# OpenSpaceAI/Nesie

Measured on AMD Instinct MI355X. Metric: ScanNet scenes/sec (fwd+bwd, 40k pts, bs=8), higher is better.
Workload: dtype f32; 1 GPU; Nesie-VoteNet supervised pretrain step (nesie-votenet-scannet-pretrain-10%): fwd+bwd+AdamW, 40000 pts/scene, fp32, random-init weights; scenes_per_gpu=8, global_batch=8, parallelism=single, world_size=1, hip_graph=True, deterministic_backward=True, index_chain_pipelined=True, forward_cu_budget=232, forward_cu_budget_from_the_head_on=248, grad_allreduce_bytes=10561936, resident_input_scenes=0

## Files before the change

nesie_amd/csrc/pwconv.hip:

```cpp
#include <algorithm>
#include "pwconv_fwd.h"
#include <stdlib.h>

namespace nesie {
PW_GEOM_DECL(4, 1, 4, 1, 1)
PW_GEOM_DECL(4, 1, 4, 1, 2)
PW_GEOM_DECL(8, 1, 4, 1, 1)
PW_GEOM_DECL(8, 1, 8, 1, 1)
PW_GEOM_DECL(9, 1, 8, 1, 1)
PW_GEOM_DECL(8, 2, 8, 1, 1)
PW_GEOM_DECL(9, 2, 8, 1, 1)
PW_GEOM_DECL(8, 4, 8, 1, 1)
int pw_launch_sparse_8_1_8_1_1(const PwFwd &a, int grid, size_t lds, hipStream_t s);

__global__ __launch_bounds__(64) void pw_stats_finalize_kernel(
    int cout, int nslots, const float *__restrict__ part, const float *__restrict__ gamma,
    const float *__restrict__ beta, float *running_mean, float *running_var, float momentum,
    float eps, float *__restrict__ coef, const float *__restrict__ chan_bias) {
  const int ch = blockIdx.x, g = ch / cout, m = ch % cout;
  const float4 *pp = (const float4 *)part + ((size_t)g * nslots) * cout + m;
  double n = 0.0, mean = 0.0, m2 = 0.0;
  auto merge = [&](double nb_, double mb_, double m2b_) {
    if (nb_ <= 0.0) return;
    const double nn = n + nb_, d = mb_ - mean;
    mean += d * (nb_ / nn);
    m2 += m2b_ + d * d * (n * nb_ / nn);
    n = nn;
  };
  auto slot = [&](const float4 q) {
    if (q.x > 0.f) {
      const double ni = q.x, mi = (double)q.y + (double)q.z / ni;
      const double m2i = (double)q.w - (double)q.z * (double)q.z / ni;
      merge(ni, mi, m2i > 0.0 ? m2i : 0.0);
    }
  };
  int i = threadIdx.x;
  for (; i + 192 < nslots; i += 256) {
    float4 q[4];
#pragma unroll
    for (int u = 0; u < 4; ++u) q[u] = pp[(size_t)(i + 64 * u) * cout];
#pragma unroll
    for (int u = 0; u < 4; ++u) slot(q[u]);
  }
  for (; i < nslots; i += 64) slot(pp[(size_t)i * cout]);
#pragma unroll
  for (int off = 32; off >= 1; off >>= 1) {
    const double nb_ = __shfl_xor(n, off, 64), mb_ = __shfl_xor(mean, off, 64), m2b_ = __shfl_xor(m2, off, 64);
    const double nn = n + nb_;
    if (nn > 0.0) {
      const double d = mb_ - mean;
      const double mm = (n * mean + nb_ * mb_) / nn;
      m2 = m2 + m2b_ + d * d * (n * nb_ / nn);
      mean = mm;
    }
    n = nn;
  }
  if (threadIdx.x != 0) return;
  const double var = n > 0.0 ? m2 / n : 0.0;
  const double invstd = 1.0 / sqrt(var + (double)eps);
  if (running_mean) {
    const double shown = mean + (chan_bias ? (double)chan_bias[ch] : 0.0);
    running_mean[ch] = (float)((1.0 - momentum) * running_mean[ch] + momentum * shown);
    const double unbiased = n > 1.0 ? var * n / (n - 1.0) : var;
    running_var[ch] = (float)((1.0 - momentum) * running_var[ch] + momentum * unbiased);
  }
  const double gm = gamma ? (double)gamma[ch] : 1.0, bt = beta ? (double)beta[ch] : 0.0;
  coef[ch * 4 + 0] = (float)(gm * invstd);
  coef[ch * 4 + 1] = (float)(bt - mean * gm * invstd);
  coef[ch * 4 + 2] = (float)mean;
  coef[ch * 4 + 3] = (float)invstd;
}

__global__ __launch_bounds__(256) void pw_pool_finish_kernel(
    long long total, int channels, int ng, int groups, int nsub, int pg, const float *__restrict__ pmax,
    const float *__restrict__ pmin, const uint8_t *__restrict__ amax,
    const uint8_t *__restrict__ amin, const float *__restrict__ coef, float lo,
    float *__restrict__ pooled, uint8_t *__restrict__ arg, float *__restrict__ zstar) {
  const long long i = (long long)blockIdx.x * 256 + threadIdx.x;
  if (i >= total) return;
  const long long row = i / groups;
  const int c = (int)((row / channels) % ng) * channels + (int)(row % channels);
  const float sc = coef ? coef[c * 4 + 0] : 1.f, bi = coef ? coef[c * 4 + 1] : 0.f;
  const bool use_min = coef && sc < 0.f;
  const float *src = use_min ? pmin : pmax;
  const uint8_t *asrc = use_min ? amin : amax;
  float e = src[i * nsub];
  int at = asrc[i * nsub];
  for (int u = 1; u < nsub; ++u) {
    const float v = src[i * nsub + u];
    const bool better = use_min ? v < e : v > e;
    at = better ? u * pg + asrc[i * nsub + u] : at;
    e = better ? v : e;
  }
  pooled[i] = coef ? fmaxf(__builtin_fmaf(e, sc, bi), lo) : e;
  arg[i] = (uint8_t)at;
  if (zstar) zstar[i] = e;
}

struct PwGeom { int kt16, kh, wr, wc, rw, pt, nhalf, per_cu; };

static bool pw_geometry(int k, int cout, PwGeom *o) {
  if (k < 1 || cout < 1 || cout > 512) return false;
  if (k <= 64) { o->kt16 = 4; o->kh = 1; }
  else if (k <= 128) { o->kt16 = 8; o->kh = 1; }
  else if (k <= 144) { o->kt16 = 9; o->kh = 1; }
  else if (k <= 256) { o->kt16 = 8; o->kh = 2; }
  else if (k <= 288) { o->kt16 = 9; o->kh = 2; }
  else if (k > 384 && k <= 512) { o->kt16 = 8; o->kh = 4; }
  else return false;
  o->nhalf = (cout + 127) / 128;
  if (o->kt16 == 4) {
    o->wr = 4; o->wc = 1; o->rw = cout <= 64 ? 1 : 2;
  } else if (cout <= 64 && o->kt16 == 8 && o->kh == 1) {
    o->wr = 4; o->wc = 1; o->rw = 1;
  } else {
    o->wr = 8; o->wc = 1; o->rw = 1;
  }
  o->pt = 64 * o->wc;
  o->per_cu = pw_per_cu(o->kt16, o->kh, o->wr * o->wc, o->wc, o->rw);
  static const int one = [] { const char *e = getenv("NESIE_PW_ONE_PER_CU"); return e ? atoi(e) : 0; }();
  if (one) o->per_cu = 1;
  return true;
}

static size_t pw_lds_bytes(const PwGeom &g) { return (size_t)2 * 16 * g.kt16 * g.pt * sizeof(float); }

}

using namespace nesie;

#ifdef PW_STAMP
long long *g_pw_stamps = nullptr;
#endif

extern "C" int nesie_pw_supported(int k, int cout, long long p) {
  PwGeom g;
  return pw_geometry(k, cout, &g) && p % g.pt == 0 && (long long)(k > cout ? k : cout) * p < (1ll << 30) ? 1 : 0;
}

static int pw_groups(const PwGeom &g, int nb, int ng, long long p) {
  const long long tiles = (long long)(nb / ng) * cdiv(p, g.pt);
  long long nwg = (long long)cu_count() * g.per_cu / (ng * g.nhalf);
  if (nwg < 1) nwg = 1;
  if (nwg > tiles) nwg = tiles;
  if (g.nhalf > 1) {
    const long long unit = 8 / std::__gcd((long long)8, (long long)ng);
    const long long r = nwg / unit * unit;
    if (r > 0 && r * 10 >= nwg * 9) nwg = r;
  }
  return (int)nwg;
}

extern "C" int nesie_pw_stat_slots(int nb, int ng, int k, int cout, long long p) {
  PwGeom g;
  if (!pw_geometry(k, cout, &g) || ng < 1) return 0;
  return pw_groups(g, nb, ng, p) * g.wc;
}

#ifdef PW_DEV
PW_GEOM_DEF(8, 2, 8, 1, 1)
PW_GEOM_DEF(8, 1, 8, 1, 1)
#endif

struct PwHost { int in_relu, rb_group, pool_group, pool_min, k4_in, sp_ns; };

static int pw_forward_impl(const char *W, PwFwd a, const PwHost &h, void *stream) {
  const int nb = a.nb, ng = a.ng, k = a.k, cout = a.cout;
  const long long p = a.p;
  NESIE_REQUIRE(nb >= 0 && ng >= 1 && k >= 1 && cout >= 1 && p >= 0, W);
  if (nb == 0 || p == 0) return NESIE_OK;
  NESIE_REQUIRE(nb % ng == 0 && (a.x || a.sp_ent) && a.w, W);
  PwGeom g;
  if (!pw_geometry(k, cout, &g) || p % g.pt != 0 || (long long)(k > cout ? k : cout) * p >= (1ll << 30)) {
    set_error("%s: %d -> %d over %lld positions is outside the built tiles", W, k, cout, p);
    return NESIE_ERR_UNSUPPORTED;
  }
  NESIE_REQUIRE(((uintptr_t)a.x & 15) == 0 && (a.x_bs & 3) == 0, W);
  NESIE_REQUIRE(!a.y || (((uintptr_t)a.y & 15) == 0 && (a.y_bs & 3) == 0), W);
  int epi = 0, pg = 16;
  if (a.in_coef) epi |= PW_AFFINE;
  if (a.y) epi |= PW_STORE;
  if (a.stat_part) epi |= PW_STATS;
  if (a.row_bias) {
    NESIE_REQUIRE(h.rb_group >= 16 && (h.rb_group & (h.rb_group - 1)) == 0 && p % h.rb_group == 0, W);
    epi |= PW_ROWBIAS;
  }
  if (a.bias) epi |= PW_BIAS;
  if (a.bn_z) {
    NESIE_REQUIRE((a.y || a.k4_gpart) && a.bn_coef && a.bn_part && ((uintptr_t)a.bn_z & 15) == 0 && (a.bnz_bs & 3) == 0, W);
    epi |= PW_BNRED;
  }
  if (h.k4_in) {
    NESIE_REQUIRE(a.k4_w && a.in_coef && k == 64 && ng == 1 && a.x_bs >= 4 * p && ((uintptr_t)a.k4_w & 15) == 0, W);
    epi |= PW_K4IN;
  }
  if (a.k4_gpart) {
    NESIE_REQUIRE(a.k4_w && a.bn_z && !a.y && cout == 64 && ng == 1 && a.bnz_bs >= 4 * p && ((uintptr_t)a.k4_w & 15) == 0 &&
                  ((uintptr_t)a.k4_gpart & 15) == 0, W);
    epi |= PW_K4Z;
  }
  if (h.pool_group) {
    NESIE_REQUIRE(h.pool_group == 16 || h.pool_group == 32, W);
    NESIE_REQUIRE(a.pool_max && a.arg_max && p % h.pool_group == 0, W);
    NESIE_REQUIRE(!h.pool_min || (a.pool_min && a.arg_min), W);
    epi |= PW_POOL | (h.pool_min ? PW_POOLMIN : 0);
    pg = h.pool_group;
  }
  if (a.sp_ent) {
    NESIE_REQUIRE(k == 128 && cout % 128 == 0 && epi == (PW_STORE | PW_BNRED) && ((uintptr_t)a.sp_ent & 7) == 0, W);
    NESIE_REQUIRE((h.sp_ns == 16 || h.sp_ns == 32 || h.sp_ns == 64) && p % 64 == 0, W);
  }
  a.sp_ns_shift = a.sp_ent ? __builtin_ctz((unsigned)h.sp_ns) : 0;
  a.sp_groups = a.sp_ent ? (int)(p / h.sp_ns) : 0;
  a.in_lo = h.in_relu ? 0.f : -__builtin_inff();
  a.rb_shift = a.row_bias ? __builtin_ctz((unsigned)h.rb_group) : 0;
  a.w_stage = 1;
  a.rev = walk_dir((long long)nb * (h.k4_in ? 4 : k) * p * 4);
#ifdef PW_STAMP
  a.stamps = g_pw_stamps;
#endif
  a.tiles_per_batch = cdiv(p, g.pt);
  a.nslots = nesie_pw_stat_slots(nb, ng, k, cout, p);
  a.nwg_g = pw_groups(g, nb, ng, p);
  a.nhalf = g.nhalf;
  const int grid = a.nwg_g * ng * g.nhalf;
  static const bool xcd_on = !(getenv("NESIE_PW_XCD") && atoi(getenv("NESIE_PW_XCD")) == 0);
  a.xcd_map = (xcd_on && g.nhalf > 1 && grid % (8 * g.nhalf) == 0) ? 1 : 0;
  const size_t lds = pw_lds_bytes(g) + (a.k4_gpart ? 2048 : 0);
  hipStream_t s = (hipStream_t)stream;
  int st = NESIE_ERR_UNSUPPORTED;
#define G(KT16, KH, WR, WC, RW)                                                          \
  if (g.kt16 == KT16 && g.kh == KH && g.wr == WR && g.wc == WC && g.rw == RW)            \
  st = PW_GEOM_NAME(KT16, KH, WR, WC, RW)(a, epi, pg, grid, lds, s)
#ifdef PW_DEV
  G(8, 2, 8, 1, 1); G(8, 1, 8, 1, 1);
#else
  if (a.sp_ent) {
    st = pw_launch_sparse_8_1_8_1_1(a, grid, lds, s);
  } else {
    G(4, 1, 4, 1, 1); G(4, 1, 4, 1, 2); G(8, 1, 4, 1, 1); G(8, 1, 8, 1, 1);
    G(9, 1, 8, 1, 1); G(8, 2, 8, 1, 1); G(9, 2, 8, 1, 1); G(8, 4, 8, 1, 1);
  }
#endif
#undef G
  if (st != NESIE_OK) {
    if (st == NESIE_ERR_UNSUPPORTED && !strstr(nesie_last_error(), "epilogue"))
      set_error("%s: no build for %d -> %d", W, k, cout);
    return st;
  }
  return check_launch(W);
}

static PwFwd pw_problem(int nb, int ng, int k, int cout, long long p, const float *x, long long x_bstride,
                        const float *w) {
  PwFwd a{};
  a.nb = nb; a.ng = ng; a.k = k; a.cout = cout; a.p = p;
  a.x = x; a.x_bs = x_bstride; a.w = w;
  return a;
}

extern "C" int nesie_pw_layer_forward(int nb, int ng, int k, int cout, long long p,
                                      const float *x, long long x_bstride, const float *w,
                                      long long w_gstride, int w_rstride, int w_cstride,
                                      const float *in_coef, int in_relu, const float *row_bias,
                                      int rb_group, const float *bias, float *y,
                                      long long y_bstride, float *stat_part, int pool_group,
                                      int pool_min, float *pool_max_out, float *pool_min_out,
                                      uint8_t *arg_max_out, uint8_t *arg_min_out, void *stream) {
  PwFwd a = pw_problem(nb, ng, k, cout, p, x, x_bstride, w);
  a.w_gs = w_gstride; a.w_rs = w_rstride; a.w_cs = w_cstride;
  a.in_coef = in_coef; a.row_bias = row_bias; a.bias = bias;
  a.y = y; a.y_bs = y_bstride; a.stat_part = stat_part;
  a.pool_max = pool_max_out; a.pool_min = pool_min_out; a.arg_max = arg_max_out; a.arg_min = arg_min_out;
  PwHost h{};
  h.in_relu = in_relu; h.rb_group = rb_group; h.pool_group = pool_group; h.pool_min = pool_min;
  return pw_forward_impl("pw_layer_forward", a, h, stream);
}

extern "C" int nesie_pw_dgrad_bn_reduce(int nb, int ng, int k, int cout, long long p,
                                        const float *x, long long x_bstride, const float *w,
                                        long long w_gstride, int w_rstride, int w_cstride,
                                        float *y, long long y_bstride, const float *bn_z,
                                        long long bnz_bstride, const float *bn_coef,
                                        float *bn_part, void *stream) {
  const char *W = "pw_dgrad_bn_reduce";
  NESIE_REQUIRE(y && bn_z && bn_coef && bn_part, W);
  PwFwd a = pw_problem(nb, ng, k, cout, p, x, x_bstride, w);
  a.w_gs = w_gstride; a.w_rs = w_rstride; a.w_cs = w_cstride;
  a.y = y; a.y_bs = y_bstride;
  a.bn_z = bn_z; a.bnz_bs = bnz_bstride; a.bn_coef = bn_coef; a.bn_part = bn_part;
  return pw_forward_impl(W, a, PwHost{}, stream);
}

extern "C" int nesie_pw_dgrad_bn_reduce_sparse(int nb, int ng, int c, int cout, long long p, int ns,
                                               const float *ent, const float *w, long long w_gstride,
                                               int w_rstride, int w_cstride, float *y,
                                               long long y_bstride, const float *bn_z,
                                               long long bnz_bstride, const float *bn_coef,
                                               float *bn_part, void *stream) {
  const char *W = "pw_dgrad_bn_reduce_sparse";
  NESIE_REQUIRE(ent && y && bn_z && bn_coef && bn_part && c == 128, W);
  PwFwd a = pw_problem(nb, ng, c, cout, p, nullptr, 0, w);
  a.w_gs = w_gstride; a.w_rs = w_rstride; a.w_cs = w_cstride;
  a.y = y; a.y_bs = y_bstride;
  a.bn_z = bn_z; a.bnz_bs = bnz_bstride; a.bn_coef = bn_coef; a.bn_part = bn_part;
  a.sp_ent = (const float2 *)ent;
  PwHost h{};
  h.sp_ns = ns;
  return pw_forward_impl(W, a, h, stream);
}

extern "C" int nesie_pw_layer_forward_k4(int nb, int cout, long long p, const float *x4,
                                         long long x4_bstride, const float *w0, const float *w,
                                         int w_rstride, int w_cstride, const float *in_coef,
                                         float *y, long long y_bstride, float *stat_part,
                                         void *stream) {
  PwFwd a = pw_problem(nb, 1, 64, cout, p, x4, x4_bstride, w);
  a.w_rs = w_rstride; a.w_cs = w_cstride;
  a.in_coef = in_coef; a.k4_w = w0;
  a.y = y; a.y_bs = y_bstride; a.stat_part = stat_part;
  PwHost h{};
  h.in_relu = 1; h.k4_in = 1;
  return pw_forward_impl("pw_layer_forward_k4", a, h, stream);
}

extern "C" int nesie_pw_dgrad_bn_reduce_k4(int nb, int k, long long p, const float *x,
                                           long long x_bstride, const float *w, int w_rstride,
                                           int w_cstride, const float *x4, long long x4_bstride,
                                           const float *w0, const float *bn_coef, float *bn_part,
                                           float *g_part, void *stream) {
  const char *W = "pw_dgrad_bn_reduce_k4";
  NESIE_REQUIRE(x4 && w0 && bn_coef && bn_part && g_part, W);
  PwFwd a = pw_problem(nb, 1, k, 64, p, x, x_bstride, w);
  a.w_rs = w_rstride; a.w_cs = w_cstride;
  a.bn_z = x4; a.bnz_bs = x4_bstride; a.bn_coef = bn_coef; a.bn_part = bn_part;
  a.k4_w = w0; a.k4_gpart = g_part;
  return pw_forward_impl(W, a, PwHost{}, stream);
}

extern "C" int nesie_pw_stats_finalize(int channels, int cout, int nslots, const float *stat_part,
                                       const float *gamma, const float *beta,
                                       float *running_mean, float *running_var, float momentum,
                                       float eps, float *coef, const float *chan_bias,
                                       void *stream) {
  const char *W = "pw_stats_finalize";
  NESIE_REQUIRE(channels >= 1 && cout >= 1 && channels % cout == 0 && nslots >= 1, W);
  NESIE_REQUIRE(stat_part && coef && (running_mean == nullptr) == (running_var == nullptr), W);
  hipLaunchKernelGGL(pw_stats_finalize_kernel, dim3(channels), dim3(64), 0, (hipStream_t)stream,
                     cout, nslots, stat_part, gamma, beta, running_mean, running_var, momentum,
                     eps, coef, chan_bias);
  return check_launch(W);
}

extern "C" int nesie_pw_pool_finish(int nb, int ng, int channels, long long p, int group, int pool_group,
                                    const float *pmax, const float *pmin, const uint8_t *amax,
                                    const uint8_t *amin, const float *coef, int relu,
                                    float *pooled, uint8_t *argmax, float *zstar, void *stream) {
  const char *W = "pw_pool_finish";
  NESIE_REQUIRE(nb >= 0 && ng >= 1 && channels >= 1 && p >= 0 && group >= 1, W);
  if (nb == 0 || p == 0) return NESIE_OK;
  NESIE_REQUIRE((pool_group == 16 || pool_group == 32) && group % pool_group == 0 && p % group == 0, W);
  NESIE_REQUIRE(group <= 256 && pmax && amax && pooled && argmax && (!coef || (pmin && amin)), W);
  const long long total = (long long)nb * channels * (p / group);
  hipLaunchKernelGGL(pw_pool_finish_kernel, dim3(cdiv(total, 256)), dim3(256), 0, (hipStream_t)stream,
                     total, channels, ng, (int)(p / group), group / pool_group, pool_group, pmax, pmin,
                     amax, amin, coef, relu ? 0.f : -__builtin_inff(), pooled, argmax, zstar);
  return check_launch(W);
}
```

nesie_amd/csrc/pwconv_fwd.h:

```cpp
#pragma once
#include "common.h"
#include <stdlib.h>
#include <string.h>
#include <type_traits>

namespace nesie {

typedef float f32x4 __attribute__((ext_vector_type(4)));
typedef float f32x2 __attribute__((ext_vector_type(2)));

template <int I, int N, class F>
__device__ __forceinline__ void static_for(F &&f) {
  if constexpr (I < N) {
    f(std::integral_constant<int, I>{});
    static_for<I + 1, N>(f);
  }
}

__device__ __forceinline__ unsigned lds_addr(const void *p) {
  return (unsigned)(uintptr_t)(__attribute__((address_space(3))) const void *)p;
}

template <int OFF>
__device__ __forceinline__ f32x4 lds_read_b128(unsigned addr) {
  static_assert(OFF >= 0 && OFF < 65536, "ds_read_b128 reach");
  f32x4 v;
  asm volatile("ds_read_b128 %0, %1 offset:%2" : "=v"(v) : "v"(addr), "n"(OFF));
  return v;
}

template <int OFF>
__device__ __forceinline__ void lds_write_b128(unsigned addr, f32x4 v) {
  static_assert(OFF >= 0 && OFF < 65536, "ds_write_b128 reach");
  asm volatile("ds_write_b128 %0, %1 offset:%2" ::"v"(addr), "v"(v), "n"(OFF) : "memory");
}

__device__ __forceinline__ f32x4 load16_saddr(unsigned voff, const void *sbase) {
  return *(const f32x4 *)((const char *)sbase + voff);
}

template <int IMM>
__device__ __forceinline__ void store16_saddr(unsigned voff, f32x4 v, void *sbase) {
  *(f32x4 *)((char *)sbase + voff + IMM) = v;
}

template <int N>
__device__ __forceinline__ void lgkm_wait() {
  asm volatile("s_waitcnt lgkmcnt(%0)" ::"n"(N) : "memory");
}

enum : int {
  PW_STORE = 1,
  PW_STATS = 2,
  PW_POOL = 4,
  PW_POOLMIN = 8,
  PW_ROWBIAS = 16,
  PW_BIAS = 32,
  PW_AFFINE = 64,
  PW_BNRED = 128,
  PW_SPARSE128 = 256,
  PW_SPARSE256 = 512,
  PW_K4IN = 1024,
  PW_K4Z = 2048,
};

__device__ __forceinline__ float k4_dot(const float4 w, float x0, float x1, float x2, float x3) {
  return __builtin_fmaf(w.w, x3, __builtin_fmaf(w.z, x2, __builtin_fmaf(w.y, x1, w.x * x0)));
}

struct PwFwd {
  const float *x; long long x_bs; long long p; int nb, k;
  const float *w; long long w_gs; int w_rs, w_cs; int ng, cout;
  const float *in_coef; float in_lo;
  float *y; long long y_bs;
  const float *row_bias; int rb_shift;
  const float *bias;
  float *stat_part; int nslots;
  float *pool_max, *pool_min; uint8_t *arg_max, *arg_min;
  const float *bn_z; long long bnz_bs;
  const float *bn_coef; float *bn_part;
  int tiles_per_batch, nwg_g, nhalf;
  int xcd_map;
  const float2 *sp_ent; int sp_ns_shift, sp_groups;
  int w_stage;
  int rev;
  const float *k4_w;
  float *k4_gpart;
  long long *stamps;
};
#ifdef PW_STAMP
#define STAMP(slot)                                                                      \
  if (a.stamps && blockIdx.x == 0 && lane == 0 && (wave == 0 || wave == 4) && iter < 24) \
    a.stamps[((wave >> 2) * 24 + iter) * 8 + (slot)] = __builtin_amdgcn_s_memtime();
#define STAMP_CLK(which)                                                     \
  if (a.stamps && blockIdx.x == 0 && threadIdx.x == 0) {                      \
    a.stamps[2 * 24 * 8 + 2 * (which)] = __builtin_amdgcn_s_memtime();       \
    a.stamps[2 * 24 * 8 + 2 * (which) + 1] = __builtin_amdgcn_s_memrealtime(); \
  }
#define STAMP_WG(which)                                                                    \
  if (a.stamps && threadIdx.x == 0 && blockIdx.x < 1024)                                    \
    a.stamps[512 + blockIdx.x * 4 + (which)] = __builtin_amdgcn_s_memrealtime();
#else
#define STAMP(slot)
#define STAMP_CLK(which)
#define STAMP_WG(which)
#endif

constexpr int pw_per_cu(int kt16, int kh, int nw, int wc, int rw) {
  const int lds = 2 * 16 * kt16 * 64 * wc * 4;
  int n = 160 * 1024 / lds;
  const int cap = nw == 4 ? (kt16 * kh * rw <= 4 ? 4 : 2) : (kt16 * kh * rw <= 8 ? 2 : 1);
  return n < cap ? n : cap;
}
constexpr int pw_min_waves(int kt16, int kh, int nw, int wc, int rw) {
  return pw_per_cu(kt16, kh, nw, wc, rw) * nw / 4;
}

template <int KT16, int KH, int WR, int WC, int RW, int EPI, int PG, bool RAGGED>
__global__ __launch_bounds__(WR *WC * 64, pw_min_waves(KT16, KH, WR *WC, WC, RW))
void pw_fwd_kernel(const PwFwd a) {
  constexpr int NW = WR * WC, NT = NW * 64, KT = 16 * KT16, KQ = KT / 4, PT = 64 * WC;
  constexpr int TILE = KT * PT, CPR = PT / 4;
  constexpr int NCH = KT * CPR;
  constexpr int NX = (NCH + NT - 1) / NT;
  constexpr bool EVEN = NCH == NX * NT;
  constexpr int ROWSTEP = NT / CPR;
  constexpr int CROWS = WR * RW * 16;
  constexpr int SPC = (EPI & PW_SPARSE128) ? 128 : (EPI & PW_SPARSE256) ? 256 : 0;
  constexpr bool K4Z = (EPI & PW_K4Z) != 0;
  static_assert(SPC % ROWSTEP == 0 && (SPC == 0 || (NCH == NX * NT && SPC <= KH * KT)), "sparse rows");
  static_assert(NT % CPR == 0 && (PG == 16 || PG == 32), "tile");
  extern __shared__ __attribute__((aligned(16))) float lds[];
  STAMP_WG(0)

  const int tid = threadIdx.x, lane = tid & 63, quad = lane >> 4, l16 = lane & 15;
  const int wave = __builtin_amdgcn_readfirstlane(tid >> 6);
  const int wr = wave / WC, wc = wave % WC;
  int half, sid;
  if (a.xcd_map) {
    const int xcd = blockIdx.x & 7, slot = blockIdx.x >> 3;
    half = slot % a.nhalf;
    sid = xcd + 8 * (slot / a.nhalf);
  } else {
    half = blockIdx.x % a.nhalf;
    sid = blockIdx.x / a.nhalf;
  }
  const int g = sid % a.ng, rank = sid / a.ng;
  const int k = a.k;
  const int c0 = half * CROWS;
  const int cout = a.cout;
  const long long p = a.p;

  const int srow = tid / CPR, scol = tid % CPR;
  auto slot_row = [](int i) constexpr { return (EVEN || i + 1 < NX) ? i * ROWSTEP : KT - ROWSTEP; };
  const unsigned voff0 = (unsigned)(((size_t)srow * p + scol * 4) * 4);
  unsigned voff_last[NX];
#pragma unroll
  for (int i = 0; i < NX; ++i) {
    int row = (KH - 1) * KT + slot_row(i) + srow;
    row = row < k ? row : k - 1;
    voff_last[i] = (unsigned)(((size_t)(row - (KH - 1) * KT) * p + scol * 4) * 4);
  }
  const unsigned lw0 = lds_addr(lds) + (unsigned)((srow * PT + scol * 4) * 4);

  float wreg[RW][KH * KQ];
  const bool w_rows = KT % 64 == 0 && (a.w_stage & 1) && a.w_cs == 1 && (a.w_rs & 3) == 0 && (a.w_gs & 3) == 0 && ((uintptr_t)a.w & 15) == 0;
  if (w_rows) {
    static_assert(WR * WC * RW * 16 <= 2 * PT, "the waves' blocks fit the two operand buffers");
    constexpr int WROWS = RW * 16, C4 = KT / 4, NL = (WROWS * C4 + 63) / 64;
    float *wl = lds + wave * (WROWS * KT);
    const int m0 = c0 + wr * WROWS;
    const float *wg0 = a.w + (size_t)g * a.w_gs + (size_t)m0 * a.w_rs;
#pragma unroll
    for (int kh = 0; kh < KH; ++kh) {
#pragma unroll
      for (int i = 0; i < NL; ++i) {
        const int f = i * 64 + lane, row = f / C4, c4 = f % C4, kcol = kh * KT + 4 * c4;
        if (NL * 64 == WROWS * C4 || f < WROWS * C4) {
          f32x4 v = (f32x4){0.f, 0.f, 0.f, 0.f};
          if (m0 + row < cout) {
            const float *src = wg0 + (size_t)row * a.w_rs + kcol;
            if (kcol + 3 < k) {
              v = *(const f32x4 *)src;
            } else {
#pragma unroll
              for (int e = 0; e < 4; ++e) v[e] = kcol + e < k ? src[e] : 0.f;
            }
          }
          *(f32x4 *)(wl + row * KT + ((4 * c4) ^ (4 * (row & 15)))) = v;
        }
      }
#pragma unroll
      for (int rw = 0; rw < RW; ++rw)
#pragma unroll
        for (int kk = 0; kk < KQ; ++kk)
          wreg[rw][kh * KQ + kk] = wl[(rw * 16 + l16) * KT + ((4 * kk + quad) ^ (4 * l16))];
    }
    __syncthreads();
  } else {
#pragma unroll
    for (int rw = 0; rw < RW; ++rw) {
      const int m = c0 + (wr * RW + rw) * 16 + l16;
      const float *wg = a.w + (size_t)g * a.w_gs + (size_t)m * a.w_rs;
#pragma unroll
      for (int kk = 0; kk < KH * KQ; ++kk) {
        const int kx = 4 * kk + quad;
        wreg[rw][kk] = (m < cout && kx < k) ? wg[(size_t)kx * a.w_cs] : 0.f;
      }
    }
  }
  float2 cof[(EPI & PW_AFFINE) ? KH : 1][(EPI & PW_AFFINE) ? NX : 1];
  if (EPI & PW_AFFINE) {
#pragma unroll
    for (int kh = 0; kh < KH; ++kh)
#pragma unroll
      for (int i = 0; i < NX; ++i) {
        int row = kh * KT + slot_row(i) + srow;
// ... 46 lines not shown
      const float *x4 = a.x + (size_t)(g + a.ng * QQ(c)) * a.x_bs + (size_t)RR(c) * PT + (size_t)i * p;
      stg[i] = load16_saddr(live ? (unsigned)(scol * 16) : 0u, live ? x4 : a.x);
      return;
    }
    const float *xb = a.x + (size_t)(g + a.ng * QQ(c)) * a.x_bs + (size_t)RR(c) * PT + (long long)(kh * KT - SPC) * p;
    if constexpr (kh < KH - 1) {
      const float *xs = live ? xb + (size_t)slot_row(i) * p : a.x;
      stg[i] = load16_saddr(live ? voff0 : 0u, xs);
    } else {
      stg[i] = load16_saddr(live ? voff_last[i] : 0u, live ? xb : a.x);
    }
  };
  auto write_slot = [&](auto ic, auto khc, int buf) {
    constexpr int i = decltype(ic)::value;
    f32x4 q = stg[i];
    if constexpr ((EPI & PW_K4IN) != 0) {
#pragma unroll
      for (int e = 0; e < 4; ++e) q[e] = k4_dot(k4w[i], stg[0][e], stg[1][e], stg[2][e], stg[3][e]);
    }
    if constexpr (K4Z) {
      if constexpr (i == 0) lds_write_b128<0>(k4z_lw + (unsigned)(buf * 1024), stx);
    }
    if constexpr (SPC > 0 && decltype(khc)::value * KT + slot_row(i) < SPC) {
      const int at = __float_as_int(q[1]) - sp_pos0;
      const float v = q[0];
      q[0] = at == 0 ? v : 0.f;
      q[1] = at == 1 ? v : 0.f;
      q[2] = at == 2 ? v : 0.f;
      q[3] = at == 3 ? v : 0.f;
    } else if constexpr ((EPI & PW_AFFINE) != 0) {
      const float2 co = cof[decltype(khc)::value][i];
      const float lo = a.in_lo;
      q[0] = fmaxf(__builtin_fmaf(q[0], co.x, co.y), lo);
      q[1] = fmaxf(__builtin_fmaf(q[1], co.x, co.y), lo);
      q[2] = fmaxf(__builtin_fmaf(q[2], co.x, co.y), lo);
      q[3] = fmaxf(__builtin_fmaf(q[3], co.x, co.y), lo);
    }
    lds_write_b128<slot_row(i) * PT * 4>(lw0 + (unsigned)(buf * TILE * 4), q);
  };

  float s1[RW], s2[RW], shift[RW];
#pragma unroll
  for (int rw = 0; rw < RW; ++rw) s1[rw] = s2[rw] = shift[rw] = 0.f;
  int ntile_done = 0;
  constexpr bool PERM = !(EPI & PW_POOL) || (EPI & (PW_STORE | PW_STATS));
  constexpr int RS = PERM ? 16 : 4;
  const int q0 = wc * 64 + (PERM ? 4 : 16) * quad;
  unsigned roff[RW];
#pragma unroll
  for (int rw = 0; rw < RW; ++rw)
    roff[rw] = (unsigned)(((size_t)(c0 + (wr * RW + rw) * 16 + l16) * p + q0) * 4);

  static_assert(!K4Z || ((EPI & PW_BNRED) && !RAGGED && WC == 1), "PW_K4Z rides on PW_BNRED");
  f32x4 zv[((EPI & PW_BNRED) && !K4Z) ? RW : 1][4];
  float4 k4zw[K4Z ? RW : 1];
  float gx[K4Z ? RW : 1][4];
  float r0[RW], r1[RW];
  float4 zc[RW];
#pragma unroll
  for (int rw = 0; rw < RW; ++rw) {
    r0[rw] = r1[rw] = 0.f;
    zc[rw] = make_float4(0.f, 0.f, 0.f, 0.f);
    if (EPI & PW_BNRED) {
      const int m = c0 + (wr * RW + rw) * 16 + l16;
      if (!RAGGED || m < cout) zc[rw] = *(const float4 *)(a.bn_coef + ((size_t)g * cout + m) * 4);
      if constexpr (K4Z) {
        k4zw[rw] = *(const float4 *)(a.k4_w + (size_t)m * 4);
#pragma unroll
        for (int j = 0; j < 4; ++j) gx[rw][j] = 0.f;
      }
    }
  }
  auto row_ok = [&](int rw) { return !RAGGED || c0 + (wr * RW + rw) * 16 + l16 < cout; };
  auto load_z = [&](int n, long long p0) {
    const float *zt = a.bn_z + (size_t)n * a.bnz_bs + p0;
    if constexpr (K4Z) return;
#pragma unroll
    for (int rw = 0; rw < RW; ++rw) {
#pragma unroll
      for (int r = 0; r < 4; ++r)
        zv[rw][r] = row_ok(rw) ? load16_saddr(roff[rw] + 4u * RS * r, zt) : (f32x4){0.f, 0.f, 0.f, 0.f};
    }
  };
  float cbias[RW], rbias[RW][4];
#pragma unroll
  for (int rw = 0; rw < RW; ++rw) {
    cbias[rw] = 0.f;
#pragma unroll
    for (int r = 0; r < 4; ++r) rbias[rw][r] = 0.f;
    if (EPI & PW_BIAS) {
      if (row_ok(rw)) cbias[rw] = a.bias[g * cout + c0 + (wr * RW + rw) * 16 + l16];
    }
  }
  auto load_row_bias = [&](int n, long long p0) {
    const size_t cols = (size_t)(p >> a.rb_shift);
#pragma unroll
    for (int rw = 0; rw < RW; ++rw)
#pragma unroll
      for (int r = 0; r < 4; ++r) {
        const size_t col = (size_t)((p0 + q0 + RS * r) >> a.rb_shift);
        rbias[rw][r] = row_ok(rw) ? a.row_bias[((size_t)n * cout + c0 + (wr * RW + rw) * 16 + l16) * cols + col] : 0.f;
      }
  };

  f32x4 acc[RW][4];
  int k4z_buf = 0;
  auto epilogue = [&](int n, long long p0) {
    float *ytile = a.y + (size_t)n * a.y_bs + p0;
    static_for<0, RW>([&](auto rwc) {
      constexpr int rw = decltype(rwc)::value;
      const int m = c0 + (wr * RW + rw) * 16 + l16;
      if (EPI & (PW_ROWBIAS | PW_BIAS)) {
        f32x4 add;
#pragma unroll
        for (int r = 0; r < 4; ++r)
          add[r] = ((EPI & PW_ROWBIAS) ? rbias[rw][r] : 0.f) + ((EPI & PW_BIAS) ? cbias[rw] : 0.f);
#pragma unroll
        for (int e = 0; e < 4; ++e) acc[rw][e] += add;
      }
      if (EPI & PW_STORE) {
        if (row_ok(rw)) {
          static_for<0, 4>([&](auto rc) {
            constexpr int r = decltype(rc)::value;
            store16_saddr<4 * RS * r>(roff[rw], (f32x4){acc[rw][0][r], acc[rw][1][r], acc[rw][2][r], acc[rw][3][r]}, ytile);
          });
        }
      }
      if constexpr (K4Z) {
        f32x4 xr[4];
        const unsigned xa = lds_addr(lds) + (unsigned)(2 * TILE * 4) + (unsigned)(k4z_buf * 1024) + (unsigned)(16 * quad);
        static_for<0, 4>([&](auto rc) {
          constexpr int r = decltype(rc)::value;
          static_for<0, 4>([&](auto jc) { xr[decltype(jc)::value] = lds_read_b128<decltype(jc)::value * 256 + r * 64>(xa); });
          lgkm_wait<0>();
          asm volatile("" : "+v"(xr[0]), "+v"(xr[1]), "+v"(xr[2]), "+v"(xr[3]));
#pragma unroll
          for (int e = 0; e < 4; ++e) {
            const float x0 = xr[0][e], x1 = xr[1][e], x2 = xr[2][e], x3 = xr[3][e];
            const float z = k4_dot(k4zw[rw], x0, x1, x2, x3);
            const float gg = __builtin_fmaf(z, zc[rw].x, zc[rw].y) > 0.f ? acc[rw][e][r] : 0.f;
            r0[rw] += gg;
            r1[rw] += gg * ((z - zc[rw].z) * zc[rw].w);
            gx[rw][0] = __builtin_fmaf(gg, x0, gx[rw][0]);
            gx[rw][1] = __builtin_fmaf(gg, x1, gx[rw][1]);
            gx[rw][2] = __builtin_fmaf(gg, x2, gx[rw][2]);
            gx[rw][3] = __builtin_fmaf(gg, x3, gx[rw][3]);
          }
          asm volatile("" :: "v"(xr[0]), "v"(xr[1]), "v"(xr[2]), "v"(xr[3]));
        });
      } else if (EPI & PW_BNRED) {
#pragma unroll
        for (int r = 0; r < 4; ++r)
#pragma unroll
          for (int e = 0; e < 4; ++e) {
            const float z = zv[rw][r][e];
            const float gg = __builtin_fmaf(z, zc[rw].x, zc[rw].y) > 0.f ? acc[rw][e][r] : 0.f;
            r0[rw] += gg;
            r1[rw] += gg * ((z - zc[rw].z) * zc[rw].w);
          }
      }
      if (EPI & PW_STATS) {
        const float first = __shfl(acc[rw][0][0], l16, 64);
        shift[rw] = ntile_done == 0 ? first : shift[rw];
#pragma unroll
        for (int r = 0; r < 4; ++r)
#pragma unroll
          for (int e = 0; e < 4; ++e) {
            const float d = acc[rw][e][r] - shift[rw];
            s1[rw] += d;
            s2[rw] += d * d;
          }
      }
      if (EPI & PW_POOL) {
        const size_t prow = (size_t)(p / PG);
        if constexpr (!PERM) {
          const size_t pcol = (size_t)((p0 + q0) / PG);
#pragma unroll
          for (int mm = 0; mm < ((EPI & PW_POOLMIN) ? 2 : 1); ++mm) {
            float ev = acc[rw][0][0];
            int at = 0;
#pragma unroll
            for (int u = 1; u < 16; ++u) {
              const float v = acc[rw][u % 4][u / 4];
              const bool better = mm ? v < ev : v > ev;
              at = better ? u : at;
              ev = better ? v : ev;
            }
            if (PG == 32) {
              at += 16 * (quad & 1);
              const float oe = __shfl_xor(ev, 16, 64);
              const int oa = __shfl_xor(at, 16, 64);
              const bool take = (mm ? oe < ev : oe > ev) || (oe == ev && oa < at);
              ev = take ? oe : ev;
              at = take ? oa : at;
            }
            if (row_ok(rw)) {
              const size_t o = ((size_t)n * cout + m) * prow + pcol;
              (mm ? a.pool_min : a.pool_max)[o] = ev;
              (mm ? a.arg_min : a.arg_max)[o] = (uint8_t)at;
            }
          }
        } else {
          constexpr int NG = 64 / PG, RPG = PG / 16;
          const size_t pcol = (size_t)((p0 + 64 * wc) / PG) + (PG == 16 ? quad : (quad & 1));
#pragma unroll
          for (int mm = 0; mm < ((EPI & PW_POOLMIN) ? 2 : 1); ++mm) {
            float ev[NG];
            int at[NG];
#pragma unroll
            for (int gi = 0; gi < NG; ++gi) {
              ev[gi] = acc[rw][0][gi * RPG];
              at[gi] = 4 * quad;
#pragma unroll
              for (int u = 1; u < 4 * RPG; ++u) {
                const int rr = u / 4, e = u % 4;
                const float v = acc[rw][e][gi * RPG + rr];
                const bool better = mm ? v < ev[gi] : v > ev[gi];
                at[gi] = better ? 16 * rr + 4 * quad + e : at[gi];
                ev[gi] = better ? v : ev[gi];
              }
            }
#pragma unroll
            for (int off = 16; off <= 32; off <<= 1) {
              float oe[NG];
              int oa[NG];
#pragma unroll
              for (int gi = 0; gi < NG; ++gi) { oe[gi] = __shfl_xor(ev[gi], off, 64); oa[gi] = __shfl_xor(at[gi], off, 64); }
#pragma unroll
              for (int gi = 0; gi < NG; ++gi) {
                const bool take = (mm ? oe[gi] < ev[gi] : oe[gi] > ev[gi]) || (oe[gi] == ev[gi] && oa[gi] < at[gi]);
                ev[gi] = take ? oe[gi] : ev[gi];
                at[gi] = take ? oa[gi] : at[gi];
              }
            }
            float sev = ev[0];
            int sat = at[0];
            const int mine = PG == 16 ? quad : (quad & 1);
#pragma unroll
            for (int gi = 1; gi < NG; ++gi) {
              sev = mine == gi ? ev[gi] : sev;
              sat = mine == gi ? at[gi] : sat;
            }
            if (row_ok(rw)) {
              const size_t o = ((size_t)n * cout + m) * prow + pcol;
              (mm ? a.pool_min : a.pool_max)[o] = sev;
              (mm ? a.arg_min : a.arg_max)[o] = (uint8_t)sat;
            }
          }
        }
      }
    });
    if (EPI & PW_STATS) ++ntile_done;
  };

  Cursor cur{rank, rank / tpb, rank % tpb, 0};
  Cursor nxt = cur;
  using KH0 = std::integral_constant<int, 0>;
  using KH1 = std::integral_constant<int, (KH > 1 ? 1 : 0)>;
  static_for<0, NX>([&](auto ic) { load_slot(ic, KH0{}, cur, cur.t < ntiles); });
#pragma unroll
  for (int rw = 0; rw < RW; ++rw)
#pragma unroll
    for (int kk = 0; kk < KH * KQ; ++kk) asm volatile("" : "+v"(wreg[rw][kk]));
  if (EPI & PW_AFFINE) {
#pragma unroll
    for (int kh = 0; kh < KH; ++kh)
#pragma unroll
      for (int i = 0; i < NX; ++i) asm volatile("" : "+v"(cof[kh][i].x), "+v"(cof[kh][i].y));
  }
  if constexpr ((EPI & PW_K4IN) != 0) {
#pragma unroll
    for (int i = 0; i < NX; ++i) asm volatile("" : "+v"(k4w[i].x), "+v"(k4w[i].y), "+v"(k4w[i].z), "+v"(k4w[i].w));
  }
#pragma unroll
  for (int rw = 0; rw < RW; ++rw) {
    if constexpr (K4Z) asm volatile("" : "+v"(k4zw[rw].x), "+v"(k4zw[rw].y), "+v"(k4zw[rw].z), "+v"(k4zw[rw].w));
    if (EPI & PW_BNRED) asm volatile("" : "+v"(zc[rw].x), "+v"(zc[rw].y), "+v"(zc[rw].z), "+v"(zc[rw].w));
    if (EPI & PW_BIAS) asm volatile("" : "+v"(cbias[rw]));
  }
  static_for<0, NX>([&](auto ic) { write_slot(ic, KH0{}, 0); });
  advance(nxt);
  static_for<0, NX>([&](auto ic) { load_slot(ic, KH1{}, nxt, nxt.t < ntiles); });
  Cursor ld = nxt;
  advance(ld);
  int buf = 0;
  int iter = 0;
  (void)iter;
  STAMP_CLK(0)
  STAMP_WG(1)
  const int chunk = PERM ? 4 * (l16 & 3) + (l16 >> 2) : l16;
  const unsigned xa0 = lds_addr(lds) + (unsigned)((quad * PT + 64 * wc + 4 * chunk) * 4);
  constexpr int PF = 2;
  auto mfma_subtile = [&](auto khc, int bufsel, auto &&stage) {
    constexpr int kh = decltype(khc)::value;
    const unsigned xa = xa0 + (unsigned)(bufsel * TILE * 4);
    f32x4 frag[PF + 1];
    auto read_frag = [&](auto kkc) {
      constexpr int kk = decltype(kkc)::value;
      constexpr int off = kk * 4 * PT * 4;
      if constexpr (off < 65536) frag[kk % (PF + 1)] = lds_read_b128<off>(xa);
      else frag[kk % (PF + 1)] = lds_read_b128<off - 65536>(xa + 65536u);
    };
    static_for<0, PF>([&](auto kc) { if constexpr (decltype(kc)::value < KQ) read_frag(kc); });
    static_for<0, KQ>([&](auto kkc) {
      constexpr int kk = decltype(kkc)::value;
      if constexpr (kk + PF < KQ) {
        read_frag(std::integral_constant<int, kk + PF>{});
        lgkm_wait<PF>();
      } else {
        lgkm_wait<(KQ - 1 - kk)>();
      }
      __builtin_amdgcn_sched_barrier(0);
      static_for<0, 4>([&](auto ec) {
        constexpr int e = decltype(ec)::value;
        static_for<0, RW>([&](auto rwc) {
          constexpr int rw = decltype(rwc)::value;
          acc[rw][e] = __builtin_amdgcn_mfma_f32_16x16x4f32(frag[kk % (PF + 1)][e], wreg[rw][kh * KQ + kk], acc[rw][e], 0, 0, 0);
        });
      });
      __builtin_amdgcn_sched_barrier(0);
      stage(kkc);
    });
  };
  auto zero_acc = [&]() {
#pragma unroll
    for (int rw = 0; rw < RW; ++rw)
#pragma unroll
      for (int e = 0; e < 4; ++e) acc[rw][e] = (f32x4){0.f, 0.f, 0.f, 0.f};
  };
  for (; cur.t < ntiles; ++iter) {
    const int n = g + a.ng * QQ(cur);
    const long long p0 = (long long)RR(cur) * PT;
    static_for<0, KH>([&](auto khc) {
      constexpr int kh = decltype(khc)::value;
      STAMP(0)
      lgkm_wait<0>();
      __builtin_amdgcn_s_barrier();
      STAMP(1)
      const bool have2 = ld.t < ntiles;
      if ((EPI & PW_BNRED) && kh == KH - 1) load_z(n, p0);
      if ((EPI & PW_ROWBIAS) && kh == KH - 1) load_row_bias(n, p0);
      if (kh == 0) zero_acc();
      constexpr int S0 = KQ - 2 - 2 * NX;
      static_assert(S0 >= 0, "staging slots do not fit the K loop");
      mfma_subtile(khc, buf, [&](auto kkc) {
        constexpr int kk = decltype(kkc)::value;
        if constexpr (kk >= S0 && (kk - S0) % 2 == 0 && (kk - S0) / 2 < NX) {
          constexpr int i = (kk - S0) / 2;
          if constexpr ((EPI & PW_K4IN) != 0) {
            if constexpr (i == 0) {
              static_for<0, NX>([&](auto jc) { write_slot(jc, std::integral_constant<int, 0>{}, buf ^ 1); });
              static_for<0, NX>([&](auto jc) { load_slot(jc, std::integral_constant<int, 0>{}, ld, have2); });
            }
          } else {
            write_slot(std::integral_constant<int, i>{}, std::integral_constant<int, (kh + 1) % KH>{}, buf ^ 1);
            load_slot(std::integral_constant<int, i>{}, std::integral_constant<int, (kh + 2) % KH>{}, ld, have2);
          }
          __builtin_amdgcn_sched_barrier(0);
        }
      });
      STAMP(2)
      if constexpr (K4Z) k4z_buf = buf;
      if (kh == KH - 1) epilogue(n, p0);
      STAMP(3)
      cur = nxt;
      nxt = ld;
      advance(ld);
      buf ^= 1;
    });
  }
  STAMP_CLK(1)
  STAMP_WG(2)
  if (EPI & PW_BNRED) {
    const int slot = rank * WC + wc;
#pragma unroll
    for (int rw = 0; rw < RW; ++rw) {
      const int m = c0 + (wr * RW + rw) * 16 + l16;
      float t0 = r0[rw], t1 = r1[rw];
      t0 += __shfl_xor(t0, 16, 64); t1 += __shfl_xor(t1, 16, 64);
      t0 += __shfl_xor(t0, 32, 64); t1 += __shfl_xor(t1, 32, 64);
      if (quad == 0 && m < cout)
        *(float2 *)(a.bn_part + (((size_t)g * cout + m) * a.nslots + slot) * 2) = make_float2(t0, t1);
      if constexpr (K4Z) {
        float4 t;
        float *tv = &t.x;
#pragma unroll
        for (int j = 0; j < 4; ++j) {
          float u = gx[rw][j];
          u += __shfl_xor(u, 16, 64);
          u += __shfl_xor(u, 32, 64);
          tv[j] = u;
        }
        if (quad == 0 && m < cout) *(float4 *)(a.k4_gpart + (((size_t)g * cout + m) * a.nslots + slot) * 4) = t;
      }
    }
  }
  if (EPI & PW_STATS) {
    const int slot = rank * WC + wc;
#pragma unroll
    for (int rw = 0; rw < RW; ++rw) {
      const int m = c0 + (wr * RW + rw) * 16 + l16;
      float t1 = s1[rw], t2 = s2[rw];
      t1 += __shfl_xor(t1, 16, 64); t2 += __shfl_xor(t2, 16, 64);
      t1 += __shfl_xor(t1, 32, 64); t2 += __shfl_xor(t2, 32, 64);
      if (quad == 0 && m < cout) {
        float4 o;
        o.x = (float)ntile_done * 64.f;
        o.y = shift[rw];
        o.z = t1; o.w = t2;
        *(float4 *)(a.stat_part + (((size_t)g * a.nslots + slot) * cout + m) * 4) = o;
      }
    }
  }
}

template <int KT16, int KH, int WR, int WC, int RW>
static int pw_launch_epi(const PwFwd &a, int epi, int pg, int grid, size_t lds, hipStream_t s) {
  const bool ragged = a.cout % (WR * RW * 16) != 0;
#define GO1(E, G, R)                                                                          \
  do {                                                                                        \
    auto kern = pw_fwd_kernel<KT16, KH, WR, WC, RW, E, G, R>;                                 \
    static bool attr = false;                                                                 \
    if (!attr) {                                                                              \
      (void)hipFuncSetAttribute((const void *)kern, hipFuncAttributeMaxDynamicSharedMemorySize, \
                                (int)lds);                                                    \
      attr = true;                                                                            \
      if (getenv("NESIE_PW_OCCUPANCY")) {      \
        int nblk = -1;                                                                        \
        (void)hipOccupancyMaxActiveBlocksPerMultiprocessor(&nblk, kern, WR * WC * 64, lds);   \
        hipFuncAttributes fa;                                                                 \
        (void)hipFuncGetAttributes(&fa, (const void *)kern);                                  \
        fprintf(stderr, "pw_fwd_kernel<%d,%d,%d,%d,%d,%d,%d,%d>: %d VGPRs, %zu B LDS, %d workgroups/CU (occupancy API), grid %d\n", \
                KT16, KH, WR, WC, RW, E, G, (int)R, fa.numRegs, lds, nblk, grid);             \
      }                                                                                       \
    }                                                                                         \
    hipLaunchKernelGGL(kern, dim3(grid), dim3(WR *WC * 64), lds, s, a);                       \
    return NESIE_OK;                                                                          \
  } while (0)
#define GO(E, G)                                                                              \
  do {                                                                                        \
    if (ragged) GO1(E, G, true); else GO1(E, G, false);                                       \
  } while (0)
#define GOW(E, G)                                                                             \
  do {                                                                                        \
    if (!ragged) GO1(E, G, false);                                                            \
  } while (0)
#ifdef PW_DEV
  if (epi == PW_STORE) GO(PW_STORE, 16);
  if (epi == (PW_STORE | PW_BNRED)) GO(PW_STORE | PW_BNRED, 16);
  if (epi == (PW_AFFINE | PW_STORE | PW_STATS)) GO(PW_AFFINE | PW_STORE | PW_STATS, 16);
  if (epi == (PW_AFFINE | PW_STORE | PW_STATS | PW_POOL | PW_POOLMIN) && pg == 16)
    GOW(PW_AFFINE | PW_STORE | PW_STATS | PW_POOL | PW_POOLMIN, 16);
  if (epi == (PW_AFFINE | PW_STORE | PW_STATS | PW_POOL | PW_POOLMIN) && pg == 32)
    GOW(PW_AFFINE | PW_STORE | PW_STATS | PW_POOL | PW_POOLMIN, 32);
  set_error("dev build");
  return NESIE_ERR_UNSUPPORTED;
#else
  if (epi & (PW_K4IN | PW_K4Z)) {
    if constexpr (KT16 == 4 && KH == 1 && WR == 4 && WC == 1 && RW == 1) {
      if (epi == (PW_K4IN | PW_AFFINE | PW_STORE | PW_STATS)) GOW(PW_K4IN | PW_AFFINE | PW_STORE | PW_STATS, 16);
      if (epi == (PW_K4Z | PW_BNRED)) GOW(PW_K4Z | PW_BNRED, 16);
    }
    set_error("pw_layer_forward: the rebuilt 4 -> 64 operand is built for 64 -> 64 layers only (0x%x)", epi);
    return NESIE_ERR_UNSUPPORTED;
  }
  const int aff = epi & PW_AFFINE;
  const int base = epi & ~PW_AFFINE;
  if (aff) {
    if (base == PW_STORE) GO(PW_AFFINE | PW_STORE, 16);
    if (base == (PW_STORE | PW_BIAS)) GO(PW_AFFINE | PW_STORE | PW_BIAS, 16);
    if (base == (PW_STORE | PW_STATS)) GO(PW_AFFINE | PW_STORE | PW_STATS, 16);
    if (base == (PW_STORE | PW_POOL) && pg == 16) GOW(PW_AFFINE | PW_STORE | PW_POOL, 16);
    if (base == PW_POOL && pg == 16) GOW(PW_AFFINE | PW_POOL, 16);
    if (base == (PW_STORE | PW_STATS | PW_POOL | PW_POOLMIN) && pg == 16)
      GOW(PW_AFFINE | PW_STORE | PW_STATS | PW_POOL | PW_POOLMIN, 16);
    if (base == (PW_STATS | PW_POOL | PW_POOLMIN) && pg == 16) GOW(PW_AFFINE | PW_STATS | PW_POOL | PW_POOLMIN, 16);
    if (base == (PW_STATS | PW_POOL | PW_POOLMIN) && pg == 32) GOW(PW_AFFINE | PW_STATS | PW_POOL | PW_POOLMIN, 32);
    if (base == (PW_STORE | PW_POOL) && pg == 32) GOW(PW_AFFINE | PW_STORE | PW_POOL, 32);
    if (base == PW_POOL && pg == 32) GOW(PW_AFFINE | PW_POOL, 32);
    if (base == (PW_STORE | PW_STATS | PW_POOL | PW_POOLMIN) && pg == 32)
      GOW(PW_AFFINE | PW_STORE | PW_STATS | PW_POOL | PW_POOLMIN, 32);
  } else {
    if (base == PW_STORE) GO(PW_STORE, 16);
    if (base == (PW_STORE | PW_BIAS)) GO(PW_STORE | PW_BIAS, 16);
    if (base == (PW_STORE | PW_BNRED)) GO(PW_STORE | PW_BNRED, 16);
    if (base == (PW_STORE | PW_STATS)) GO(PW_STORE | PW_STATS, 16);
    if (base == (PW_STORE | PW_STATS | PW_ROWBIAS)) GOW(PW_STORE | PW_STATS | PW_ROWBIAS, 16);
  }
  set_error("pw_layer_forward: epilogue combination 0x%x (pool group %d) is not built", epi, pg);
  return NESIE_ERR_UNSUPPORTED;
#endif
#undef GO
#undef GOW
#undef GO1
}

template <int KT16, int KH, int WR, int WC, int RW, int EPI>
static int pw_launch_sparse(const PwFwd &a, int grid, size_t lds, hipStream_t s) {
  auto kern = pw_fwd_kernel<KT16, KH, WR, WC, RW, EPI, 16, false>;
  static bool attr = false;
  if (!attr) {
    (void)hipFuncSetAttribute((const void *)kern, hipFuncAttributeMaxDynamicSharedMemorySize, (int)lds);
    attr = true;
  }
  hipLaunchKernelGGL(kern, dim3(grid), dim3(WR * WC * 64), lds, s, a);
  return NESIE_OK;
}

#define PW_GEOM_NAME(KT16, KH, WR, WC, RW) pw_launch_##KT16##_##KH##_##WR##_##WC##_##RW
#define PW_GEOM_DECL(KT16, KH, WR, WC, RW) \
  int PW_GEOM_NAME(KT16, KH, WR, WC, RW)(const PwFwd &a, int epi, int pg, int grid, size_t lds, hipStream_t s);
#define PW_GEOM_DEF(KT16, KH, WR, WC, RW)                                                        \
  namespace nesie {                                                                             \
  int PW_GEOM_NAME(KT16, KH, WR, WC, RW)(const PwFwd &a, int epi, int pg, int grid, size_t lds, \
                                         hipStream_t s) {                                       \
    return pw_launch_epi<KT16, KH, WR, WC, RW>(a, epi, pg, grid, lds, s);                       \
  }                                                                                             \
  }

}
```

nesie_amd/csrc/pwconv_g10.hip:

```cpp
#include "pwconv_fwd.h"
namespace nesie {
int pw_launch_sparse_8_1_8_1_1(const PwFwd &a, int grid, size_t lds, hipStream_t s) {
  return pw_launch_sparse<8, 1, 8, 1, 1, PW_STORE | PW_BNRED | PW_SPARSE128>(a, grid, lds, s);
}
}
```

Before: 687.1 scenes/s.

## Replace sparse dgrad pointwise launch with warp-specialized tail kernel

Swaps the templated sparse 8/1/8 pointwise-conv dgrad path for a dedicated 1024-thread kernel. Eight producer waves compact sparse entries per tile into LDS lists with ballot/popcount and gather weights from an LDS-resident weight block. Eight consumer waves prefetch BN z values, apply the BN-reduce epilogue and store outputs, with tiles double-buffered in LDS. The aim is to exploit sparsity directly and overlap the gather compute with the epilogue memory traffic. The cost is high LDS use and one block per CU, plus barriers every tile that couple the two halves.

```diff
diff --git a/nesie_amd/csrc/pwconv.hip b/nesie_amd/csrc/pwconv.hip
--- a/nesie_amd/csrc/pwconv.hip
+++ b/nesie_amd/csrc/pwconv.hip
@@ -11,7 +11,7 @@
 PW_GEOM_DECL(8, 2, 8, 1, 1)
 PW_GEOM_DECL(9, 2, 8, 1, 1)
 PW_GEOM_DECL(8, 4, 8, 1, 1)
-int pw_launch_sparse_8_1_8_1_1(const PwFwd &a, int grid, size_t lds, hipStream_t s);
+int pw_tail_dgrad_launch(const PwFwd &a, int grid, hipStream_t s);
 
 __global__ __launch_bounds__(64) void pw_stats_finalize_kernel(
     int cout, int nslots, const float *__restrict__ part, const float *__restrict__ gamma,
@@ -236,7 +236,7 @@
   G(8, 2, 8, 1, 1); G(8, 1, 8, 1, 1);
 #else
   if (a.sp_ent) {
-    st = pw_launch_sparse_8_1_8_1_1(a, grid, lds, s);
+    st = pw_tail_dgrad_launch(a, grid, s);
   } else {
     G(4, 1, 4, 1, 1); G(4, 1, 4, 1, 2); G(8, 1, 4, 1, 1); G(8, 1, 8, 1, 1);
     G(9, 1, 8, 1, 1); G(8, 2, 8, 1, 1); G(9, 2, 8, 1, 1); G(8, 4, 8, 1, 1);
diff --git a/nesie_amd/csrc/pwconv_fwd.h b/nesie_amd/csrc/pwconv_fwd.h
--- a/nesie_amd/csrc/pwconv_fwd.h
+++ b/nesie_amd/csrc/pwconv_fwd.h
@@ -63,6 +63,17 @@
   PW_K4IN = 1024,
   PW_K4Z = 2048,
 };
+
+__device__ __forceinline__ void pw_bnred_step(float z, float y, const float4 zc, float &r0, float &r1) {
+  const float gg = __builtin_fmaf(z, zc.x, zc.y) > 0.f ? y : 0.f;
+  r0 += gg;
+  r1 += gg * ((z - zc.z) * zc.w);
+}
+__device__ __forceinline__ float pw_bnred_quads(float t) {
+  t += __shfl_xor(t, 16, 64);
+  t += __shfl_xor(t, 32, 64);
+  return t;
+}
 
 __device__ __forceinline__ float k4_dot(const float4 w, float x0, float x1, float x2, float x3) {
   return __builtin_fmaf(w.w, x3, __builtin_fmaf(w.z, x2, __builtin_fmaf(w.y, x1, w.x * x0)));
@@ -415,12 +426,7 @@
 #pragma unroll
         for (int r = 0; r < 4; ++r)
 #pragma unroll
-          for (int e = 0; e < 4; ++e) {
-            const float z = zv[rw][r][e];
-            const float gg = __builtin_fmaf(z, zc[rw].x, zc[rw].y) > 0.f ? acc[rw][e][r] : 0.f;
-            r0[rw] += gg;
-            r1[rw] += gg * ((z - zc[rw].z) * zc[rw].w);
-          }
+          for (int e = 0; e < 4; ++e) pw_bnred_step(zv[rw][r][e], acc[rw][e][r], zc[rw], r0[rw], r1[rw]);
       }
       if (EPI & PW_STATS) {
         const float first = __shfl(acc[rw][0][0], l16, 64);
@@ -639,9 +645,7 @@
 #pragma unroll
     for (int rw = 0; rw < RW; ++rw) {
       const int m = c0 + (wr * RW + rw) * 16 + l16;
-      float t0 = r0[rw], t1 = r1[rw];
-      t0 += __shfl_xor(t0, 16, 64); t1 += __shfl_xor(t1, 16, 64);
-      t0 += __shfl_xor(t0, 32, 64); t1 += __shfl_xor(t1, 32, 64);
+      const float t0 = pw_bnred_quads(r0[rw]), t1 = pw_bnred_quads(r1[rw]);
       if (quad == 0 && m < cout)
         *(float2 *)(a.bn_part + (((size_t)g * cout + m) * a.nslots + slot) * 2) = make_float2(t0, t1);
       if constexpr (K4Z) {
diff --git a/nesie_amd/csrc/pwconv_g10.hip b/nesie_amd/csrc/pwconv_g10.hip
--- a/nesie_amd/csrc/pwconv_g10.hip
+++ /dev/null
@@ -1,6 +0,0 @@
-#include "pwconv_fwd.h"
-namespace nesie {
-int pw_launch_sparse_8_1_8_1_1(const PwFwd &a, int grid, size_t lds, hipStream_t s) {
-  return pw_launch_sparse<8, 1, 8, 1, 1, PW_STORE | PW_BNRED | PW_SPARSE128>(a, grid, lds, s);
-}
-}
diff --git a/nesie_amd/csrc/pwconv_tail_dgrad.hip b/nesie_amd/csrc/pwconv_tail_dgrad.hip
--- /dev/null
+++ b/nesie_amd/csrc/pwconv_tail_dgrad.hip
@@ -0,0 +1,167 @@
+#include "pwconv_fwd.h"
+
+namespace nesie {
+
+constexpr int TD_C = 128, TD_K = 128;
+constexpr int TD_PITCH = 68;
+constexpr int TD_TILE = TD_K * TD_PITCH;
+constexpr int TD_LIST = 192;
+constexpr size_t TD_LDS = (size_t)(TD_C * TD_K + 2 * TD_TILE) * sizeof(float) + (size_t)8 * TD_LIST * sizeof(float2);
+
+__device__ __forceinline__ void td_barrier() {
+  lgkm_wait<0>();
+  __builtin_amdgcn_s_barrier();
+  asm volatile("" ::: "memory");
+}
+
+__device__ __forceinline__ int td_rank(unsigned long long m) {
+  return (int)__builtin_amdgcn_mbcnt_hi((unsigned)(m >> 32), __builtin_amdgcn_mbcnt_lo((unsigned)m, 0u));
+}
+
+__global__ __launch_bounds__(1024, 1) void pw_tail_dgrad_kernel(const PwFwd a) {
+  extern __shared__ __attribute__((aligned(16))) float lds[];
+  float *wl = lds;
+  float *yt = lds + TD_C * TD_K;
+  const int tid = threadIdx.x, lane = tid & 63;
+  const int wave = __builtin_amdgcn_readfirstlane(tid >> 6);
+  const int half = blockIdx.x % a.nhalf, sid = blockIdx.x / a.nhalf;
+  const int g = sid % a.ng, rank = sid / a.ng;
+  const int c0 = half * TD_K, cout = a.cout;
+  const long long p = a.p;
+  const int tpb = a.tiles_per_batch, nwg = a.nwg_g, nq = a.nb / a.ng;
+  const int ntiles = nq * tpb;
+
+  {
+    const float *wg = a.w + (size_t)g * a.w_gs + (size_t)c0 * a.w_rs;
+    for (int i = tid; i < TD_C * TD_K; i += 1024) {
+      const int c = i / TD_K, k = i % TD_K;
+      wl[i] = wg[(size_t)k * a.w_rs + (size_t)c * a.w_cs];
+    }
+  }
+  td_barrier();
+
+  auto where = [&](int t, int &n, long long &p0) {
+    const int q = t / tpb, r = t % tpb;
+    n = g + a.ng * (a.rev ? nq - 1 - q : q);
+    p0 = (long long)(a.rev ? tpb - 1 - r : r) * 64;
+  };
+
+  if (wave < 8) {
+    const int qt = wave >> 1, kh = (wave & 1) * 64;
+    const int base = (16 * qt) & ((1 << a.sp_ns_shift) - 1);
+    auto entries = [&](int t) {
+      int n; long long p0;
+      where(t, n, p0);
+      return a.sp_ent + ((size_t)n * a.sp_groups + (size_t)((p0 + 16 * qt) >> a.sp_ns_shift)) * TD_C + lane;
+    };
+    float2 elo = make_float2(0.f, 0.f), ehi = elo;
+    if (rank < ntiles) { const float2 *e = entries(rank); elo = e[0]; ehi = e[64]; }
+    float2 *list = (float2 *)(yt + 2 * TD_TILE) + wave * TD_LIST;
+    const char *wk = (const char *)(wl + kh + lane);
+    int it = 0;
+    for (int t = rank; t < ntiles; t += nwg, ++it) {
+      const float vlo = elo.x, vhi = ehi.x;
+      const int atlo = __float_as_int(elo.y) - base, athi = __float_as_int(ehi.y) - base;
+      if (t + nwg < ntiles) { const float2 *e = entries(t + nwg); elo = e[0]; ehi = e[64]; }
+#pragma unroll
+      for (int i = 0; i < TD_LIST / 128; ++i) *(f32x4 *)&list[2 * (i * 64 + lane)] = (f32x4){0.f, 0.f, 0.f, 0.f};
+      if (TD_LIST % 128 != 0 && lane < (TD_LIST % 128) / 2)
+        *(f32x4 *)&list[2 * ((TD_LIST / 128) * 64 + lane)] = (f32x4){0.f, 0.f, 0.f, 0.f};
+      asm volatile("" ::: "memory");
+      int offs[17], slo = -1, shi = -1, off = 0;
+#pragma unroll
+      for (int j = 0; j < 16; ++j) {
+        const unsigned long long mlo = __builtin_amdgcn_ballot_w64(atlo == j), mhi = __builtin_amdgcn_ballot_w64(athi == j);
+        const int nlo = __builtin_popcountll(mlo);
+        slo = atlo == j ? off + td_rank(mlo) : slo;
+        shi = athi == j ? off + nlo + td_rank(mhi) : shi;
+        offs[j] = off;
+        off += (nlo + __builtin_popcountll(mhi) + 3) & ~3;
+      }
+      offs[16] = off;
+      if (slo >= 0) list[slo] = make_float2(vlo, __int_as_float(lane * TD_K * 4));
+      if (shi >= 0) list[shi] = make_float2(vhi, __int_as_float((lane + 64) * TD_K * 4));
+      asm volatile("" ::: "memory");
+      float *yb = yt + (it & 1) * TD_TILE + (kh + lane) * TD_PITCH + 16 * qt;
+      const f32x4 *l4 = (const f32x4 *)list;
+      f32x4 ea = l4[0], eb = l4[1];
+      int at = 2;
+#pragma unroll
+      for (int r = 0; r < 4; ++r) {
+        f32x4 yv;
+#pragma unroll
+        for (int jj = 0; jj < 4; ++jj) {
+          float acc = 0.f;
+          for (int i = offs[4 * r + jj]; i < offs[4 * r + jj + 1]; i += 4) {
+            const float w0 = *(const float *)(wk + __float_as_int(ea[1])), w1 = *(const float *)(wk + __float_as_int(ea[3]));
+            const float w2 = *(const float *)(wk + __float_as_int(eb[1])), w3 = *(const float *)(wk + __float_as_int(eb[3]));
+            const float v0 = ea[0], v1 = ea[2], v2 = eb[0], v3 = eb[2];
+            ea = l4[at];
+            eb = l4[at + 1];
+            at += 2;
+            acc = __builtin_fmaf(v0, w0, acc);
+            acc = __builtin_fmaf(v1, w1, acc);
+            acc = __builtin_fmaf(v2, w2, acc);
+            acc = __builtin_fmaf(v3, w3, acc);
+          }
+          yv[jj] = acc;
+        }
+        *(f32x4 *)(yb + 4 * r) = yv;
+      }
+      td_barrier();
+    }
+  } else {
+    const int quad = lane >> 4, m = c0 + (wave - 8) * 16 + (lane & 15);
+    const float4 zc = *(const float4 *)(a.bn_coef + ((size_t)g * cout + m) * 4);
+    const unsigned roff = (unsigned)(((size_t)m * p + 4 * quad) * 4);
+    const float *yl = yt + ((wave - 8) * 16 + (lane & 15)) * TD_PITCH + 4 * quad;
+    float r0 = 0.f, r1 = 0.f;
+    auto load_z = [&](int t, f32x4 (&z)[4]) {
+      int n; long long p0;
+      where(t, n, p0);
+      const float *zt = a.bn_z + (size_t)n * a.bnz_bs + p0;
+#pragma unroll
+      for (int r = 0; r < 4; ++r) z[r] = load16_saddr(roff + 64u * r, zt);
+    };
+    auto tile = [&](int t, int it, f32x4 (&zv)[4], f32x4 (&zn)[4]) {
+      if (t + nwg < ntiles) load_z(t + nwg, zn);
+      td_barrier();
+      int n; long long p0;
+      where(t, n, p0);
+      float *ytile = a.y + (size_t)n * a.y_bs + p0;
+      const float *yb = yl + (it & 1) * TD_TILE;
+      f32x4 y[4];
+#pragma unroll
+      for (int r = 0; r < 4; ++r) y[r] = *(const f32x4 *)(yb + 16 * r);
+#pragma unroll
+      for (int r = 0; r < 4; ++r)
+#pragma unroll
+        for (int e = 0; e < 4; ++e) pw_bnred_step(zv[r][e], y[r][e], zc, r0, r1);
+      static_for<0, 4>([&](auto rc) { store16_saddr<64 * decltype(rc)::value>(roff, y[decltype(rc)::value], ytile); });
+    };
+    f32x4 za[4], zb[4];
+    if (rank < ntiles) load_z(rank, za);
+    int it = 0;
+    for (int t = rank; t < ntiles;) {
+      tile(t, it, za, zb);
+      t += nwg; ++it;
+      if (t >= ntiles) break;
+      tile(t, it, zb, za);
+      t += nwg; ++it;
+    }
+    const float t0 = pw_bnred_quads(r0), t1 = pw_bnred_quads(r1);
+    if (quad == 0) *(float2 *)(a.bn_part + (((size_t)g * cout + m) * a.nslots + rank) * 2) = make_float2(t0, t1);
+  }
+}
+
+int pw_tail_dgrad_launch(const PwFwd &a, int grid, hipStream_t s) {
+  static bool attr = false;
+  if (!attr) {
+    (void)hipFuncSetAttribute((const void *)pw_tail_dgrad_kernel, hipFuncAttributeMaxDynamicSharedMemorySize, (int)TD_LDS);
+    attr = true;
+  }
+  hipLaunchKernelGGL(pw_tail_dgrad_kernel, dim3(grid), dim3(1024), TD_LDS, s, a);
+  return NESIE_OK;
+}
+
+}
```

After: 689.6 scenes/s, median of 4. Within noise of the previous version (+0.4%).
